# MILAB-IIT-CV/ATDN_vSLAM

Measured on AMD Instinct MI355X. Metric: frame-pairs/sec, KITTI 1241x376 odometry inference at 1/2/4/8 MI355X, higher is better.
Workload: dtype f32 via 3xf16 split MFMA (fp32 accumulate); 1 GPU; KITTI seq-03-shaped 376x1241 uint8 frames (resident in HBM) resized to 376x1232, GMA flow 12 GRU iters + CLVO head -> 6-DoF trajectory (BASELINE configs[1]); streams_per_gpu=2, gru_iters=12, parallelism=pairs sharded x1, one all-gather of 512-d features, replicated LSTM scan

## Files before the change

atdn_vslam_amd/_lib.py:

```python
import ctypes as C
import os

_HERE = os.path.dirname(os.path.abspath(__file__))
LIB_PATH = os.environ.get("ATDN_LIB_PATH") or os.path.join(_HERE, "libatdn_hip.so")

_f32p = C.POINTER(C.c_float)
_i64p = C.POINTER(C.c_int64)
_vp = C.c_void_p

SIGNATURES = {
    "atdn_version": (C.c_int, []),
    "atdn_last_error": (C.c_char_p, []),
    "atdn_gma_create": (C.c_int, [C.POINTER(_vp), C.c_int, C.c_int, C.c_int, C.c_int]),
    "atdn_gma_set_low_latency": (C.c_int, [_vp, C.c_int]),
    "atdn_gma_load": (C.c_int, [_vp, C.c_char_p, _vp, _i64p, C.c_int]),
    "atdn_gma_finalize": (C.c_int, [_vp]),
    "atdn_gma_forward": (C.c_int, [_vp, _vp, _vp, C.c_int, C.c_int, _vp, _vp, _vp, _vp]),
    "atdn_gma_forward_predictions": (C.c_int, [_vp, _vp, _vp, C.c_int, C.c_int, _vp, _vp, _vp]),
    "atdn_gma_forward_sequence": (C.c_int, [_vp, _vp, C.c_int, C.c_int, _vp, _vp, _vp, _vp]),
    "atdn_gma_forward_sequence_continued": (C.c_int, [_vp, _vp, C.c_int, C.c_int, _vp, _vp, _vp, _vp]),
    "atdn_gma_debug_read": (C.c_long, [_vp, C.c_char_p, _vp, C.c_long, _vp]),
    "atdn_gma_profile": (C.c_int, [_vp, C.c_int, C.c_int, C.c_int, _f32p, _vp]),
    "atdn_gma_profile_mode": (C.c_int, [_vp, C.c_int, C.c_int, C.c_int, C.c_int, _f32p, _vp]),
    "atdn_gma_set_range_probe": (C.c_int, [_vp, C.c_int]),
# ... 35 lines not shown
    "atdn_ingest_destroy": (None, [_vp]),
    "atdn_flow_pack_f16": (C.c_int, [_vp, C.c_int, C.c_int, C.c_int, C.c_int, C.c_int, _vp, _vp]),
    "atdn_flow_gather_clips": (C.c_int, [_vp, C.c_int, C.c_int, C.c_int, _vp, _vp, C.c_int, C.c_int, _vp, _vp]),
    "atdn_map_search": (C.c_int, [_vp, C.c_int, C.c_int, _vp, C.c_int, C.c_int, _vp, _vp, _vp]),
    "atdn_map_gather_images_u8": (C.c_int, [_vp, C.c_int, C.c_long, _vp, C.c_int, _vp, _vp]),
    "atdn_corr_lookup": (C.c_int, [_vp, _vp, _vp, _vp, C.c_int, C.c_int, C.c_int, _vp, _vp, C.c_int, _vp]),
    "atdn_corr_pyramid": (C.c_int, [_vp, _vp, C.c_int, C.c_int, C.c_int, C.c_int, _vp, _vp, _vp, _vp, _vp]),
    "atdn_corr_lookup_bricks": (C.c_int, [_vp, _vp, C.c_int, C.c_int, C.c_int, C.c_int, _vp, _vp, _vp, _vp, _vp, _vp, _vp, _vp,
                                          _vp, _vp]),
    "atdn_conv2d_nhwc": (C.c_int, [_vp, C.c_int, C.c_int, C.c_int, C.c_int, _vp, _vp, C.c_int, C.c_int, C.c_int,
                                   C.c_int, C.c_int, C.c_int, C.c_int, _vp, _vp]),
    "atdn_conv2d_nhwc_sf": (C.c_int, [_vp, C.c_int, C.c_int, C.c_int, C.c_int, _vp, _vp, C.c_int, C.c_int, C.c_int,
                                      C.c_int, C.c_int, C.c_int, _vp, _vp]),
    "atdn_conv2d_nhwc_sf_epi": (C.c_int, [_vp, C.c_int, C.c_int, C.c_int, C.c_int, _vp, _vp, C.c_int, C.c_int, C.c_int,
                                      C.c_int, C.c_int, C.c_int, C.c_int, _vp, _vp]),
}

GMA_STAGES = ("fnet", "corr", "pool", "cnet", "attention", "lookup", "motion_encoder", "aggregate", "gru_zr", "gru_q",
              "flow_head", "mask", "gru_ctx", "attn_logits", "agg_vt", "convc1", "gru_zr_v", "gru_q_v")

_lib = None


def lib():
    global _lib
    if _lib is None:
        if not os.path.exists(LIB_PATH):
            raise RuntimeError(
                "%s is missing: the HIP extension has not been built (python -m atdn_vslam_amd.build). "
                "There is no CPU fallback for the product path." % LIB_PATH)
# ... 31 lines not shown
```

atdn_vslam_amd/csrc/capi.hip:

```cpp
#include "../../include/atdn_hip.h"

#include <cmath>
#include <cstring>

#include "clvo.h"
#include "gma.h"
#include "vae.h"
#include "clvo_train.h"
#include "frontend.h"
#include "conv_sf.h"
#include "epilogues_sf.h"

namespace atdn {
extern template TileChoice conv_dispatch<MODE_TAP, EpiBias<ACT_NONE>>(const ConvShape&, EpiBias<ACT_NONE>, hipStream_t);
extern template TileChoice conv_dispatch<MODE_TAP, EpiBias<ACT_RELU>>(const ConvShape&, EpiBias<ACT_RELU>, hipStream_t);
extern template TileChoice conv_dispatch<MODE_ROW, EpiBias<ACT_NONE>>(const ConvShape&, EpiBias<ACT_NONE>, hipStream_t);
extern template TileChoice conv_dispatch<MODE_ROW, EpiBias<ACT_RELU>>(const ConvShape&, EpiBias<ACT_RELU>, hipStream_t);
extern template TileChoice conv_dispatch<MODE_TAP, EpiScale>(const ConvShape&, EpiScale, hipStream_t);

extern template TileChoice conv_sf_dispatch<EpiBias<ACT_NONE>>(const ConvShape&, float, EpiBias<ACT_NONE>, hipStream_t);
extern template TileChoice conv_sf_dispatch<SfBias<ACT_NONE>>(const ConvShape&, float, SfBias<ACT_NONE>, hipStream_t);

static thread_local std::string g_last_error;
void set_last_error(const std::string& msg) { g_last_error = msg; }
}
// ... 560 lines not shown
    (void)hipFree(tmp);
    A.release();
    throw;
  }
  (void)hipFree(tmp);
  A.release();
  ATDN_API_END
}

int atdn_conv2d_nhwc_sf(const float* src, int nimg, int H, int W, int Cin, const float* weight_host,
                        const float* bias_host, int Cout, int KH, int KW, int stride, int padH, int padW, float* dst,
                        void* stream) {
  return atdn_conv2d_nhwc_sf_epi(src, nimg, H, W, Cin, weight_host, bias_host, Cout, KH, KW, stride, padH, padW, 0, dst, stream);
}

}
```

atdn_vslam_amd/csrc/conv_sf6.h:

```cpp
#pragma once
#include <cstdlib>
#include <type_traits>
#include "conv_sf.h"

namespace atdn {

struct Conv2Geom {
  const float* src0; const float* src1;
  long sb0, sb1;
  int ld0, ld1, C0, C1;
  int H, W, Ho, Wo;
  int KH, KW, padH, padW;
  int PH, PW;
  int tiles_x, tiles_y;
  int nimg, ntile_n;
  const float* w; int ldw; int N;
  float wscale;
  const float* in_mean; const float* in_rstd;
};

inline bool conv_halo_eligible(const ConvShape& s) {
  if (s.stride != 1 || s.wb != 0) return false;
  return (s.KH == 3 && s.KW == 3) || (s.KH == 1 && s.KW == 5) || (s.KH == 5 && s.KW == 1);
}

template <class E, class = void> struct epi_gen6 : std::integral_constant<int, 0> {};
template <class E> struct epi_gen6<E, std::void_t<decltype(E::kGen6)>> : std::integral_constant<int, E::kGen6> {};
template <class E, class = void> struct EpiAux4 { struct type {}; };
template <class E> struct EpiAux4<E, std::void_t<typename E::Aux4>> { using type = typename E::Aux4; };
template <class E, class = void> struct epi_flowhead : std::false_type {};
template <class E> struct epi_flowhead<E, std::void_t<decltype(E::kFlowHead)>> : std::bool_constant<E::kFlowHead> {};
template <class E, class = void> struct epi_ring3 : std::false_type {};
template <class E> struct epi_ring3<E, std::void_t<decltype(E::kRing3)>> : std::bool_constant<E::kRing3> {};
template <class E, class = void> struct epi_rawacc : std::false_type {};
// ... 19 lines not shown
  constexpr int TM = TH * TW / 32 / WM, TN = BN / 32 / WN;
  static_assert(TM * WM * 32 == TH * TW && TN * WN * 32 == BN, "wave grid must tile the block");
  static_assert(32 % TW == 0 || TW % 32 == 0, "a 32-pixel MFMA row tile must cover whole tile rows");
  constexpr int NTAP = KH * KW;
  constexpr int RSTEP = NT / 8;
  constexpr int PROWS = (TH + KH - 1) * (TW + KW - 1);
  constexpr int PW = TW + KW - 1;
  constexpr int NP = (PROWS + RSTEP - 1) / RSTEP;
  constexpr int ROWB = 160;
  constexpr int RS = PW * ROWB;
  constexpr bool SWAP = epi_vec4<Epi>::value;
  constexpr int PSZ = (TH + KH - 1) * RS;
  __shared__ __attribute__((aligned(256))) char Pbytes[NIMG * PSZ];

  const int tid = threadIdx.x;
  const int tiles_img = g.tiles_x * g.tiles_y;
  const int nblk = g.nimg * tiles_img * g.ntile_n;
  const int id = xcd_remap(bidx, nblk);
  const int tile_n = id % g.ntile_n;
  const int tmg = id / g.ntile_n;
  const int img = tmg / tiles_img;
  const int tloc = tmg - img * tiles_img;
  const int ty0 = (tloc / g.tiles_x) * TH, tx0 = (tloc % g.tiles_x) * TW;
  const int n0 = tile_n * BN;
  const int lane = tid & 63, wave = tid >> 6;
#ifdef ATDN_CONV_STAMP
  constexpr int kStamp = conv_stamp_kind<Epi>::value;
  unsigned long long st_r0 = 0, st_t0 = 0, st_t1 = 0, st_t2 = 0, st_bar = 0;
  unsigned long long st_e_slab = 0, st_e_wait = 0, st_e_apply = 0;
  if constexpr (kStamp >= 0) { st_r0 = __builtin_amdgcn_s_memrealtime(); st_t0 = __builtin_amdgcn_s_memtime(); }
#endif

  const int jrow = (tid >> 3) & 7;
  const int s = tid & 7, r0 = !NORM ? tid >> 3 : ((tid >> 6) << 3) + 2 * (jrow & 1) + ((jrow >> 1) & 1) + 4 * (jrow >> 2);
  static_assert((TH + KH - 1) * RS / 16 <= 4096, "LDS offset field");
  unsigned pmeta[NP];
#pragma unroll
  for (int k = 0; k < NP; ++k) {
    const int prow = r0 + RSTEP * k;
    unsigned off = 0;
    const int py = prow / PW, px = prow - py * PW;
    if (prow < PROWS) {
      const int iy = ty0 - g.padH + py, ix = tx0 - g.padW + px;
      if ((unsigned)iy < (unsigned)g.H && (unsigned)ix < (unsigned)g.W) off = (unsigned)(iy * g.W + ix) + 1u;
    }
    pmeta[k] = (off << 12) | (unsigned)((py * RS + px * ROWB + 16 * s) >> 4);
    if (prow >= PROWS) pmeta[k] = pmeta[0];
  }
  const float* s0 = g.src0 + (long)img * g.sb0;
  const float* s1 = g.src1 ? g.src1 + (long)img * g.sb1 : nullptr;
  const int nck = (g.C0 + g.C1) >> 5;

  float4 pr[NP];
  auto fetch_patch = [&](int c) {
    const int cc = c << 5;
    const float* sp; int ld, co;
    if (cc < g.C0) { sp = s0; ld = g.ld0; co = cc; } else { sp = s1; ld = g.ld1; co = cc - g.C0; }
#pragma unroll
    for (int k = 0; k < NP; ++k)
      pr[k] = *reinterpret_cast<const float4*>(sp + (long)((pmeta[k] >> 12) ? (pmeta[k] >> 12) - 1 : 0) * ld + co + 4 * s);
  };
  auto store_patch = [&](int buf) {
// ... 22 lines not shown
    *reinterpret_cast<uint2*>(px + 64 + 8 * s) = make_uint2(l0, l1);
  };

  const int wm = wave / WN, wn = wave % WN;
  SfAcc acc[TM][TN];
#pragma unroll
  for (int i = 0; i < TM; ++i)
#pragma unroll
    for (int j = 0; j < TN; ++j) {
#pragma unroll
      for (int e = 0; e < 16; ++e) acc[i][j].b[e >> 3][(e >> 2) & 1][e & 3] = 0.f;
    }
  {
    const int n16 = lane & 15, g16 = lane >> 4;
    int a_off[TM];
#pragma unroll
    for (int i = 0; i < TM; ++i) a_off[i] = ((wm * TM + i) * 2) * RS + n16 * ROWB + 16 * g16;
    const char* Pb = Pbytes;
    const int nblk16 = (g.N + 15) >> 4;
    const float* wrow[TN][2];
#pragma unroll
    for (int j = 0; j < TN; ++j)
#pragma unroll
      for (int cb = 0; cb < 2; ++cb)
        wrow[j][cb] = g.w + (long)min(((n0 >> 4) + (wn * TN + j) * 2 + cb), nblk16 - 1) * (NTAP * nck) * 512 + lane * 4;
    constexpr int RT = (NTAP % 3 == 0 || epi_ring3<Epi>::value) ? 3 : 2;
    constexpr int CU = (NTAP % RT == 0) ? 1 : RT;
    constexpr int NS = CU * NTAP;
    static_assert(NS % RT == 0, "ring size must divide the K steps of an unrolled iteration");
    struct WFrag { f16x8 hi[TN][2], lo[TN][2]; };
    WFrag wr[RT];
    auto load_w = [&](WFrag& f, int c0, int st, int cb) __attribute__((always_inline)) {
// ... 10 lines not shown
#pragma unroll
    for (int st = 0; st < RT - 1; ++st) { load_w(wr[st], 0, st, 0); load_w(wr[st], 0, st, 1); }
    if constexpr ((ABL & 1) != 0) { load_w(wr[RT - 1], 0, RT - 1, 0); load_w(wr[RT - 1], 0, RT - 1, 1); }
    if constexpr (NORM) {
#pragma unroll
      for (int k = 0; k < NP; ++k) store_row_norm(0, k, nmu, nrs);
    } else {
      store_patch(0);
    }
    __syncthreads();
#ifdef ATDN_CONV_STAMP
    if constexpr (kStamp >= 0) st_t1 = __builtin_amdgcn_s_memtime();
#endif
    f16x8 ah[2][TM], al[2][TM];
    auto read_a = [&](int half, int tap) __attribute__((always_inline)) {
      const char* arow = Pb + (tap / KW + half) * RS + (tap % KW) * ROWB;
#pragma unroll
      for (int i = 0; i < TM; ++i) {
        ah[half][i] = *reinterpret_cast<const f16x8*>(arow + a_off[i]);
        if constexpr (!FAST) al[half][i] = *reinterpret_cast<const f16x8*>(arow + a_off[i] + 64);
      }
    };
    auto mfma_half = [&](int half, const WFrag& w) __attribute__((always_inline)) {
#pragma unroll
      for (int i = 0; i < TM; ++i)
#pragma unroll
        for (int j = 0; j < TN; ++j)
#pragma unroll
          for (int cb = 0; cb < 2; ++cb) {
            f32x4v c = acc[i][j].b[half][cb];
// ... 52 lines not shown
              else if (k - ((hs + 1 < NH) ? nds : 0) < nvm) __builtin_amdgcn_sched_group_barrier(0x020, 1, 0);
              else if (k - ((hs + 1 < NH) ? nds : 0) - nvm < ndw) __builtin_amdgcn_sched_group_barrier(0x200, 1, 0);
            }
          }
        }
        if (!(ABL & 2)) {
#ifdef ATDN_CONV_STAMP
          unsigned long long st_b0 = 0;
          if constexpr (kStamp >= 0) { asm volatile("s_waitcnt lgkmcnt(0)" ::: "memory"); st_b0 = __builtin_amdgcn_s_memtime(); }
#endif
          asm volatile("s_waitcnt lgkmcnt(0)\n\ts_barrier" ::: "memory");
#ifdef ATDN_CONV_STAMP
          if constexpr (kStamp >= 0) st_bar += __builtin_amdgcn_s_memtime() - st_b0;
#endif
          Pb = Pbytes + ((c + 1) & 1) * PSZ;
        }
        if (!(ABL & 4)) read_a(0, 0);
      }
    }
  }

#ifdef ATDN_CONV_STAMP
  if constexpr (kStamp >= 0) st_t2 = __builtin_amdgcn_s_memtime();
  auto stamp_out = [&]() __attribute__((always_inline)) {
    if constexpr (kStamp >= 0) {
      asm volatile("s_waitcnt vmcnt(0) lgkmcnt(0)" ::: "memory");
      const unsigned long long t3 = __builtin_amdgcn_s_memtime(), r1 = __builtin_amdgcn_s_memrealtime();
      const unsigned hw = __builtin_amdgcn_s_getreg((31 << 11) | 4), xcc = __builtin_amdgcn_s_getreg((31 << 11) | 20);
      if (wave == 0 && lane == 0 && bidx < ATDN_CONV_STAMP_SLOTS) {
        unsigned long long* o = atdn_conv_stamps_dev[kStamp * 2 + (KH == 5 ? 1 : 0)][bidx];
        o[0] = st_r0; o[1] = r1; o[2] = st_t1 - st_t0; o[3] = st_t2 - st_t1; o[4] = st_bar; o[5] = t3 - st_t2;
        o[6] = ((unsigned long long)xcc << 32) | hw; o[7] = t3 - st_t0;
        o[8] = st_e_slab; o[9] = st_e_wait; o[10] = st_e_apply; o[11] = 0;
      }
    }
  };
#endif
  if constexpr (KH != 3 || !Epi::kStats) __builtin_amdgcn_s_setprio(0);
  if constexpr (NORM) sf_report(norm_sat);
  if constexpr ((ABL & 8) != 0) {
    float tot = 0.f;
#pragma unroll
    for (int i = 0; i < TM; ++i)
#pragma unroll
      for (int j = 0; j < TN; ++j)
#pragma unroll
        for (int e = 0; e < 16; ++e) tot += acc[i][j].b[e >> 3][(e >> 2) & 1][e & 3];
    if (tot == 1.2345e-30f) ep(img, 0, 0, tot);
    return;
  }
  if constexpr (SWAP) {
    static_assert(NW * 32 * LDS_LD * 4 <= NIMG * PSZ, "transpose slabs must fit in the patch images");
    __syncthreads();
    float* tb = reinterpret_cast<float*>(Pbytes) + wave * (32 * LDS_LD);
    const int trow = lane >> 3, tcol = (lane & 7) * 4;
    auto tile_pixel = [&](int i, int q) {
      const int p = (wm * TM + i) * 32 + 8 * q + trow;
      const int oy = ty0 + p / TW, ox = tx0 + p % TW;
      if constexpr ((ABL & 16) != 0) return p;
      return (oy < g.Ho && ox < g.Wo) ? oy * g.Wo + ox : -1;
    };
    constexpr bool RAW = epi_rawacc<Epi>::value && !epi_flowhead<Epi>::value;
    auto slab_write = [&](const SfAcc& a) __attribute__((always_inline)) {
      const float sc = RAW ? 1.0f : g.wscale;
#pragma unroll
      for (int hh = 0; hh < 2; ++hh)
#pragma unroll
        for (int cb = 0; cb < 2; ++cb)
          *reinterpret_cast<float4*>(tb + (16 * hh + (lane & 15)) * LDS_LD + 16 * cb + 4 * (lane >> 4)) =
              RAW ? make_float4(a.b[hh][cb][0], a.b[hh][cb][1], a.b[hh][cb][2], a.b[hh][cb][3])
                  : make_float4(a.b[hh][cb][0] * sc, a.b[hh][cb][1] * sc, a.b[hh][cb][2] * sc, a.b[hh][cb][3] * sc);
    };
    if constexpr (epi_flowhead<Epi>::value) {
      static_assert(!epi_flowhead<Epi>::value || (WM == 1 && TN == 1 && TW == 16), "one block holds all output channels of its pixels");
      constexpr int RP = 20;
// ... 47 lines not shown
              d1 = __builtin_amdgcn_mfma_f32_16x16x32_f16(w2l[1], xh[pb], d1, 0, 0, 0);
            }
            d0 = __builtin_amdgcn_mfma_f32_16x16x32_f16(w2h[0], xh[pb], d0, 0, 0, 0);
            d1 = __builtin_amdgcn_mfma_f32_16x16x32_f16(w2h[1], xh[pb], d1, 0, 0, 0);
            float* rp = tb + (16 * pb + n16) * RP;
            *reinterpret_cast<float4*>(rp + 4 * g16) = make_float4(d0[0] * ep.w2inv, d0[1] * ep.w2inv, d0[2] * ep.w2inv, d0[3] * ep.w2inv);
            if (g16 == 0) *reinterpret_cast<float2*>(rp + 16) = make_float2(d1[0] * ep.w2inv, d1[1] * ep.w2inv);
          }
          __syncthreads();
          for (int idx = tid; idx < 32 * 18; idx += NT) {
            const int px = idx / 18, u = idx - px * 18;
            const float* rq = reinterpret_cast<const float*>(Pbytes) + px * RP + u;
            float sum = 0.f;
#pragma unroll
            for (int w = 0; w < NW; ++w) sum += rq[w * (32 * LDS_LD)];
            const int p = i * 32 + px;
            const int oy = ty0 + p / TW, ox = tx0 + p % TW;
            if (oy < g.Ho && ox < g.Wo)
              ep.G[(long)(n0 / (NW * 32)) * ep.gstride + ((long)img * ep.npix + (long)oy * g.Wo + ox) * 18 + u] = sum;
          }
          __syncthreads();
        }
        sf_report(sat);
        return;
      }
    }
    struct NoAux {};
    using AuxT = typename std::conditional<Epi::kPrefetch, typename EpiAux4<Epi>::type, NoAux>::type;
    constexpr bool PIPE = Epi::kPrefetch && sizeof(AuxT) <= 2 * sizeof(float4);
    AuxT aux_next[PIPE ? 4 : 1];
    bool clamped = false;
    if constexpr (PIPE) {
      const int nb0 = n0 + (wn * TN) * 32 + tcol;
#pragma unroll
// ... 93 lines not shown
#pragma unroll
  for (int j = 0; j < TN; ++j)
#pragma unroll
    for (int cs = 0; cs < NSET; ++cs) {
      const int n = min(n0 + (wn * TN + j) * 32 + col_of(cs), g.N - 1);
      biasj[j][cs] = 0.f;
      if constexpr (Epi::kStats) biasj[j][cs] = ep.bias[n];
      if constexpr (epi_bias_arg<Epi>::value) colj[j][cs] = ep.col(n);
    }
#pragma unroll
  for (int i = 0; i < TM; ++i) {
    const int pbase = (wm * TM + i) * 32;
    int mm[NPX];
#pragma unroll
    for (int e = 0; e < NPX; ++e) {
      const int p = pbase + pix_of(e);
      const int oy = ty0 + p / TW, ox = tx0 + p % TW;
      mm[e] = (oy < g.Ho && ox < g.Wo) ? oy * g.Wo + ox : -1;
    }
    int cnt = 0;
    unsigned mo[NPX];
    if constexpr (Epi::kStats) {
#pragma unroll
      for (int e = 0; e < NPX; ++e) {
        cnt += mm[e] >= 0 ? 1 : 0;
        mo[e] = (unsigned)max(mm[e], 0) * (unsigned)ep.ld;
      }
      cnt += __shfl_xor(cnt, 16);
      cnt += __shfl_xor(cnt, 32);
      cnt = __builtin_amdgcn_readfirstlane(cnt);
    }
    const bool full = cnt == 32;
    const float inv_cnt = 1.0f / (float)(cnt > 0 ? cnt : 1);
// ... 71 lines not shown
}

template <int TH, int TW, int BN, int WM, int WN, int KH, int KW, class Epi, bool FAST = false, bool NORM = false, int ABL = 0>
__global__ __launch_bounds__(WM * WN * 64, 1) void conv_sf6_kernel(const Conv2Geom g, const Epi ep) {
  conv_sf6_body<TH, TW, BN, WM, WN, KH, KW, Epi, FAST, NORM, ABL>(g, ep, (int)blockIdx.x);
}

__device__ __forceinline__ Conv2Geom conv2_geom_pick(const Conv2Geom& a, const Conv2Geom& b, bool s) {
  Conv2Geom g;
  g.src0 = s ? b.src0 : a.src0; g.src1 = s ? b.src1 : a.src1; g.sb0 = s ? b.sb0 : a.sb0; g.sb1 = s ? b.sb1 : a.sb1;
  g.ld0 = s ? b.ld0 : a.ld0; g.ld1 = s ? b.ld1 : a.ld1; g.C0 = s ? b.C0 : a.C0; g.C1 = s ? b.C1 : a.C1;
  g.H = s ? b.H : a.H; g.W = s ? b.W : a.W; g.Ho = s ? b.Ho : a.Ho; g.Wo = s ? b.Wo : a.Wo;
  g.KH = s ? b.KH : a.KH; g.KW = s ? b.KW : a.KW; g.padH = s ? b.padH : a.padH; g.padW = s ? b.padW : a.padW;
  g.PH = s ? b.PH : a.PH; g.PW = s ? b.PW : a.PW; g.tiles_x = s ? b.tiles_x : a.tiles_x; g.tiles_y = s ? b.tiles_y : a.tiles_y;
  g.nimg = s ? b.nimg : a.nimg; g.ntile_n = s ? b.ntile_n : a.ntile_n;
  g.w = s ? b.w : a.w; g.ldw = s ? b.ldw : a.ldw; g.N = s ? b.N : a.N; g.wscale = s ? b.wscale : a.wscale;
  g.in_mean = nullptr; g.in_rstd = nullptr;
  return g;
}
template <int TH, int TW, int BN, int WM, int WN, int KH, int KW, class Epi, bool FAST = false>
__global__ __launch_bounds__(WM * WN * 64, 1) void conv_sf6_pair_kernel(const Conv2Geom g0, const Conv2Geom g1, const Epi ep0,
                                                                        const Epi ep1, const int nblk0, const int start1) {
  const int b = (int)blockIdx.x;
  if (b >= nblk0 && b < start1) return;
  const bool second = b >= start1;
  const Conv2Geom g = conv2_geom_pick(g0, g1, second);
  const Epi ep = Epi::pick(ep0, ep1, second);
  conv_sf6_body<TH, TW, BN, WM, WN, KH, KW, Epi, FAST, false, 0>(g, ep, second ? b - start1 : b);
}

// ... 3 lines not shown
  ATDN_CHECK(s.KH == KH && s.KW == KW && s.stride == 1, "kernel shape does not match the instantiation");
  Conv2Geom g{};
  g.src0 = s.src0; g.src1 = s.src1; g.sb0 = s.sb0; g.sb1 = s.sb1; g.ld0 = s.ld0; g.ld1 = s.ld1;
  g.C0 = s.C0; g.C1 = s.C1; g.H = s.H; g.W = s.W;
  g.KH = s.KH; g.KW = s.KW; g.padH = s.padH; g.padW = s.padW;
  g.Ho = conv_out(s.H, s.KH, 1, s.padH); g.Wo = conv_out(s.W, s.KW, 1, s.padW);
  g.PH = TH + s.KH - 1; g.PW = TW + s.KW - 1;
  ATDN_CHECK(s.C0 % 32 == 0 && s.C1 % 32 == 0 && s.C0 > 0 && s.ld0 % 4 == 0, "TAP-mode channel constraints");
  ATDN_CHECK(s.ldw % 4 == 0 && s.ldw >= s.KH * s.KW * (s.C0 + s.C1), "weight rows too short");
  ATDN_CHECK(!epi_vec4<Epi>::value || !Epi::kPrefetch || s.N % 4 == 0, "channel-vector epilogue with operand loads needs N % 4 == 0");
  ATDN_CHECK((long)s.H * s.W < (1L << 20) - 1, "image too large for the packed patch descriptor");
  ATDN_CHECK((long)g.Ho * g.Wo * 1024L * 4L <= (1L << 32) && s.ld0 <= 1024 && s.ld1 <= 1024 && s.N <= 1024,
             "per-image slice of 4 GB or more: the 32-bit epilogue offsets would wrap");
  g.tiles_x = cdiv(g.Wo, TW); g.tiles_y = cdiv(g.Ho, TH);
  g.nimg = s.nimg; g.ntile_n = cdiv(s.N, BN);
  g.w = s.wfrag16; g.ldw = s.ldw; g.N = s.N; g.wscale = wscale;
  g.in_mean = s.in_mean; g.in_rstd = s.in_rstd;
  ATDN_CHECK(NORM == (s.in_mean != nullptr) && (!NORM || (s.in_rstd && s.C1 == 0 && s.ld0 == s.C0)),
             "normalise-on-load: one dense fp32 source with its mean / rstd");
  ATDN_CHECK(g.w != nullptr, "missing weight copy for this kernel");
  return g;
}

template <int TH, int BN, int WM, int WN, int KH, int KW, class Epi, bool FAST = false, bool NORM = false, int ABL = 0>
inline void launch_conv_sf6(const ConvShape& s, float wscale, Epi ep, hipStream_t st) {
  constexpr int TW = 16;
  const Conv2Geom g = conv_sf6_geom<TH, BN, WM, WN, KH, KW, Epi, FAST, NORM, ABL>(s, wscale);
  set_groups(ep, g.tiles_x * g.tiles_y * (TH * TW / 32));
  const int nblk = g.nimg * g.tiles_x * g.tiles_y * g.ntile_n;
  hipLaunchKernelGGL((conv_sf6_kernel<TH, TW, BN, WM, WN, KH, KW, Epi, FAST, NORM, ABL>), dim3(nblk), dim3(WM * WN * 64), 0, st, g, ep);
  ATDN_HIP(hipGetLastError());
}

template <int TH, int BN, int WM, int WN, int KH, int KW, class Epi, bool FAST>
inline void launch_conv_sf6_pair(const ConvShape& s0, float wscale0, Epi ep0, const ConvShape& s1, float wscale1, Epi ep1,
                                 hipStream_t st) {
  constexpr int TW = 16;
  static_assert(!Epi::kStats, "the pair launch serves plain-store epilogues");
  const Conv2Geom g0 = conv_sf6_geom<TH, BN, WM, WN, KH, KW, Epi, FAST, false, 0>(s0, wscale0);
  const Conv2Geom g1 = conv_sf6_geom<TH, BN, WM, WN, KH, KW, Epi, FAST, false, 0>(s1, wscale1);
  const int nblk0 = g0.nimg * g0.tiles_x * g0.tiles_y * g0.ntile_n;
  const int start1 = (nblk0 + 7) / 8 * 8;
  const int nblk1 = g1.nimg * g1.tiles_x * g1.tiles_y * g1.ntile_n;
  hipLaunchKernelGGL((conv_sf6_pair_kernel<TH, TW, BN, WM, WN, KH, KW, Epi, FAST>), dim3(start1 + nblk1), dim3(WM * WN * 64), 0, st,
                     g0, g1, ep0, ep1, nblk0, start1);
  ATDN_HIP(hipGetLastError());
}


inline int conv_sf6_block_width_3x3(const ConvShape& s) {
  const int Ho = conv_out(s.H, s.KH, 1, s.padH), Wo = conv_out(s.W, s.KW, 1, s.padW);
  const long tiles = (long)s.nimg * cdiv(Wo, 16) * cdiv(Ho, 8);
  int bn = 64;
  if (s.N <= 32) bn = 32;
  else if (s.N == 96) bn = 96;
  else {
    int best = cdiv(s.N, 64) * 64;
    for (int c : {128, 256})
// ... 129 lines not shown
```

atdn_vslam_amd/csrc/gma.hip:

```cpp
#include "gma.h"
#include "small_convs.h"
#include "conv_sf.h"
#include "epilogues_sf.h"

namespace atdn { const float* zero_line(); }

namespace atdn {

extern template TileChoice conv_dispatch<MODE_TAP, EpiBias<ACT_NONE>>(const ConvShape&, EpiBias<ACT_NONE>, hipStream_t);
extern template TileChoice conv_dispatch<MODE_TAP, EpiBias<ACT_RELU>>(const ConvShape&, EpiBias<ACT_RELU>, hipStream_t);
extern template TileChoice conv_dispatch<MODE_ROW, EpiBias<ACT_RELU>>(const ConvShape&, EpiBias<ACT_RELU>, hipStream_t);
extern template TileChoice conv_dispatch<MODE_TAP, EpiBiasStats>(const ConvShape&, EpiBiasStats, hipStream_t);
extern template TileChoice conv_dispatch<MODE_ROW, EpiBiasStats>(const ConvShape&, EpiBiasStats, hipStream_t);
extern template TileChoice conv_dispatch<MODE_TAP, EpiBiasReluAddRelu>(const ConvShape&, EpiBiasReluAddRelu, hipStream_t);
extern template TileChoice conv_dispatch<MODE_TAP, EpiContextSplit>(const ConvShape&, EpiContextSplit, hipStream_t);
extern template TileChoice conv_dispatch<MODE_TAP, EpiScale>(const ConvShape&, EpiScale, hipStream_t);
extern template TileChoice conv_dispatch<MODE_TAP, EpiQK>(const ConvShape&, EpiQK, hipStream_t);
extern template TileChoice conv_dispatch<MODE_TAP, EpiStoreT>(const ConvShape&, EpiStoreT, hipStream_t);
extern template TileChoice conv_dispatch<MODE_TAP, EpiAggregate>(const ConvShape&, EpiAggregate, hipStream_t);
extern template TileChoice conv_dispatch<MODE_TAP, EpiGruZR>(const ConvShape&, EpiGruZR, hipStream_t);
extern template TileChoice conv_dispatch<MODE_TAP, EpiGruQ>(const ConvShape&, EpiGruQ, hipStream_t);
extern template TileChoice conv_dispatch<MODE_TAP, EpiFlowDelta>(const ConvShape&, EpiFlowDelta, hipStream_t);

extern template TileChoice conv_dispatch<MODE_ROW, SfBias<ACT_RELU>>(const ConvShape&, SfBias<ACT_RELU>, hipStream_t);
// ... 301 lines not shown
  z_.alloc(n8 * 128); rh_.alloc(n8 * 128); fh_.alloc(n8 * 256); mask_.alloc(n8 * 576);
  if (sf) fhG_.alloc(2 * n8 * 18);
  coords1_.alloc(n8 * 2); flow4_.alloc(n8 * 4);
  if (sf) for (int p = 0; p < 2; ++p) { pre_zr_[p].alloc(n8 * 256); pre_q_[p].alloc(n8 * 128); }
  ATDN_HIP(hipMemset(corrfeat_.p, 0, corrfeat_.n * sizeof(float)));
  ATDN_HIP(hipMemset(vT_.p, 0, vT_.n * sizeof(float)));
  ATDN_HIP(hipMemset(attn_.p, 0, attn_.n * sizeof(float)));
  ATDN_HIP(hipMemset(flow4_.p, 0, flow4_.n * sizeof(float)));
  ATDN_HIP(hipDeviceSynchronize());
  ws_bytes_ = 0;
  DeviceBuf* all[] = {&img4_, &enc_[0], &enc_[1], &enc_[2], &enc_[3], &fmap_, &psum_, &pm2_, &pyr_[0], &pyr_[1], &pyr_[2],
                      &pyr_[3], &h_[0], &h_[1], &x_, &qk_, &attn_, &vT_, &corrfeat_, &cor1_, &corflo_, &flo1_, &z_,
                      &rh_, &fh_, &mask_, &coords1_, &flow4_};
  for (auto* b : all) ws_bytes_ += (size_t)b->n * sizeof(float);
  (void)zero_line();
  sf_counter_attach();
  ATDN_HIP(hipStreamCreateWithFlags(&cap_stream_, hipStreamNonBlocking));
  ready_ = true;
}

void GmaNet::run_encoder(const EncoderWeights& E, bool instance, int nimg, hipStream_t st, float** out_buf, int* outH,
                         int* outW) {
  int h = conv_out(H, 7, 2, 3), w = conv_out(W, 7, 2, 3);
  float* P = enc_[0].p; float* Q = enc_[1].p; float* R = enc_[2].p;
  auto stats_conv = [&](auto mode_tag, const PackedConv& L, const float* src, int ld, int ih, int iw, int stride,
                        int pad, float* dst, int slot) {
    constexpr int MODE = decltype(mode_tag)::value;
    ConvShape s = conv_shape(L, src, ld, (long)ih * iw * ld, nimg, ih, iw, stride, pad, pad);
    const int oh = conv_out(ih, L.KH, stride, pad), ow = conv_out(iw, L.KW, stride, pad);
    EpiBiasStats ep{L.b, dst, (long)oh * ow * L.N, L.N, psum_.p, pm2_.p, 0};
// ... 604 lines not shown
```

include/atdn_hip.h:

```cpp
#ifndef ATDN_HIP_H
#define ATDN_HIP_H

#include <stddef.h>
#include <stdint.h>

#ifdef __cplusplus
extern "C" {
#endif

typedef struct atdn_gma atdn_gma;
typedef struct atdn_clvo atdn_clvo;
typedef struct atdn_vae atdn_vae;
typedef struct atdn_clvo_trainer atdn_clvo_trainer;

int atdn_version(void);
const char* atdn_last_error(void);


#define ATDN_PRECISION_F32 0
#define ATDN_PRECISION_SPLIT_F16 1
#define ATDN_PRECISION_F16 2
int atdn_gma_create(atdn_gma** out, int H, int W, int max_batch, int precision);

int atdn_gma_set_low_latency(atdn_gma* h, int on);
// ... 101 lines not shown
int atdn_corr_lookup_bricks(const float* fmap1, const float* fmap2, int B, int H8, int W8, int C, const float* coords,
                            float* pyr0, float* pyr1, float* pyr2, float* pyr3, float* samples,
                            const float* convc1_weight_host, const float* convc1_bias_host, float* cor1, void* stream);

int atdn_conv2d_nhwc(const float* src, int nimg, int H, int W, int Cin, const float* weight_host,
                     const float* bias_host, int Cout, int KH, int KW, int stride, int padH, int padW, int relu,
                     float* dst, void* stream);

int atdn_conv2d_nhwc_sf(const float* src, int nimg, int H, int W, int Cin, const float* weight_host,
                        const float* bias_host, int Cout, int KH, int KW, int stride, int padH, int padW, float* dst,
                        void* stream);
int atdn_conv2d_nhwc_sf_epi(const float* src, int nimg, int H, int W, int Cin, const float* weight_host,
                            const float* bias_host, int Cout, int KH, int KW, int stride, int padH, int padW, int sf_store,
                            float* dst, void* stream);

#ifdef __cplusplus
}
#endif
#endif
```

Baseline: 418.1 frame-pairs/s.

## Use precomputed fitted tile plans for ragged edges in halo-patch convs

Adds a host-built tile plan that covers the output image with full 16xTH tiles plus reshaped edge tiles sized to the remainder strips, cached on device per shape. For plain-store epilogues without stats or normalisation, the halo-patch conv kernel reads its tile geometry from the plan and uses variable patch strides and pixel-slot mappings. The aim is to cut the wasted MFMA work and patch loads that partially empty edge tiles spend on out-of-range pixels. In exchange each block does a plan load, float-reciprocal index math and more address arithmetic, and the A-fragment addressing becomes more complex.

```diff
diff --git a/atdn_vslam_amd/_lib.py b/atdn_vslam_amd/_lib.py
--- a/atdn_vslam_amd/_lib.py
+++ b/atdn_vslam_amd/_lib.py
@@ -73,6 +73,7 @@
                                       C.c_int, C.c_int, C.c_int, _vp, _vp]),
     "atdn_conv2d_nhwc_sf_epi": (C.c_int, [_vp, C.c_int, C.c_int, C.c_int, C.c_int, _vp, _vp, C.c_int, C.c_int, C.c_int,
                                       C.c_int, C.c_int, C.c_int, C.c_int, _vp, _vp]),
+    "atdn_conv_tile_plan": (C.c_int, [C.c_int, C.c_int, C.c_int, C.c_int, C.c_int, C.POINTER(C.c_int), C.c_int, C.POINTER(C.c_int)]),
 }
 
 GMA_STAGES = ("fnet", "corr", "pool", "cnet", "attention", "lookup", "motion_encoder", "aggregate", "gru_zr", "gru_q",
diff --git a/atdn_vslam_amd/csrc/capi.hip b/atdn_vslam_amd/csrc/capi.hip
--- a/atdn_vslam_amd/csrc/capi.hip
+++ b/atdn_vslam_amd/csrc/capi.hip
@@ -9,6 +9,7 @@
 #include "clvo_train.h"
 #include "frontend.h"
 #include "conv_sf.h"
+#include "conv_tile_plan.h"
 #include "epilogues_sf.h"
 
 namespace atdn {
@@ -599,4 +600,17 @@
   return atdn_conv2d_nhwc_sf_epi(src, nimg, H, W, Cin, weight_host, bias_host, Cout, KH, KW, stride, padH, padW, 0, dst, stream);
 }
 
-}
+int atdn_conv_tile_plan(int Ho, int Wo, int TH, int KH, int KW, int* tiles, int capacity, int* count) {
+  ATDN_API_BEGIN
+  ATDN_CHECK(Ho >= 1 && Wo >= 1 && count && capacity >= 0 && (tiles || capacity == 0), "bad argument");
+  ATDN_CHECK(TH == 4 || TH == 8 || TH == 12, "tile heights of the halo-patch kernels: 4, 8, 12");
+  ATDN_CHECK((KH == 3 && KW == 3) || (KH == 1 && KW == 5) || (KH == 5 && KW == 1), "kernel shapes of the halo-patch kernels: 3x3, 1x5, 5x1");
+  const std::vector<ConvTile> plan = conv_tile_plan(Ho, Wo, TH, KH, KW);
+  *count = (int)plan.size();
+  for (int i = 0; i < (int)plan.size() && i < capacity; ++i) {
+    tiles[4 * i + 0] = plan[i].y0; tiles[4 * i + 1] = plan[i].x0; tiles[4 * i + 2] = plan[i].h; tiles[4 * i + 3] = plan[i].w;
+  }
+  ATDN_API_END
+}
+
+}
diff --git a/atdn_vslam_amd/csrc/conv_sf6.h b/atdn_vslam_amd/csrc/conv_sf6.h
--- a/atdn_vslam_amd/csrc/conv_sf6.h
+++ b/atdn_vslam_amd/csrc/conv_sf6.h
@@ -2,6 +2,7 @@
 #include <cstdlib>
 #include <type_traits>
 #include "conv_sf.h"
+#include "conv_tile_plan.h"
 
 namespace atdn {
 
@@ -17,7 +18,10 @@
   const float* w; int ldw; int N;
   float wscale;
   const float* in_mean; const float* in_rstd;
+  const ConvTile* plan; int ntiles;
 };
+
+template <class Epi, bool NORM, int ABL> struct conv_sf6_fit : std::bool_constant<!Epi::kStats && !NORM && ABL == 0> {};
 
 inline bool conv_halo_eligible(const ConvShape& s) {
   if (s.stride != 1 || s.wb != 0) return false;
@@ -67,14 +71,43 @@
   __shared__ __attribute__((aligned(256))) char Pbytes[NIMG * PSZ];
 
   const int tid = threadIdx.x;
-  const int tiles_img = g.tiles_x * g.tiles_y;
+  constexpr bool FIT = conv_sf6_fit<Epi, NORM, ABL>::value;
+  const int tiles_img = FIT ? g.ntiles : g.tiles_x * g.tiles_y;
   const int nblk = g.nimg * tiles_img * g.ntile_n;
   const int id = xcd_remap(bidx, nblk);
   const int tile_n = id % g.ntile_n;
   const int tmg = id / g.ntile_n;
   const int img = tmg / tiles_img;
   const int tloc = tmg - img * tiles_img;
-  const int ty0 = (tloc / g.tiles_x) * TH, tx0 = (tloc % g.tiles_x) * TW;
+  int ty0, tx0, t_h = TH, t_w = TW, t_wh = TW, t_hh = TH / 2, t_ry = 2, t_dy = 1, t_dx = 0, pwf = PW;
+  float inv_wh = 1.0f / TW;
+  auto load_tile = [&]() __attribute__((always_inline)) {
+    const int4 ta = reinterpret_cast<const int4*>(g.plan)[2 * tloc], tb4 = reinterpret_cast<const int4*>(g.plan)[2 * tloc + 1];
+    ty0 = ta.x; tx0 = ta.y; t_h = ta.z; t_w = ta.w; t_wh = tb4.x; t_hh = tb4.y;
+    t_ry = tb4.z & 255; t_dy = (tb4.z >> 8) & 255; t_dx = (tb4.z >> 16) & 255;
+    inv_wh = __int_as_float(__builtin_amdgcn_readfirstlane(__float_as_int(__builtin_amdgcn_rcpf((float)t_wh))));
+  };
+  if constexpr (FIT) {
+    load_tile();
+    pwf = (t_dx ? 2 * t_wh : t_w) + KW - 1;
+  } else {
+    ty0 = (tloc / g.tiles_x) * TH; tx0 = (tloc % g.tiles_x) * TW;
+  }
+  const int rs = FIT ? pwf * ROWB : RS;
+  const int hoff = FIT ? t_dy * rs + t_dx * ROWB : RS;
+  const int nprow = FIT ? ((t_ry == 2 ? (t_h + 1) & ~1 : t_h) + KH - 1) * pwf : PROWS;
+  const float inv_pw = __builtin_amdgcn_rcpf((float)pwf);
+  auto slot_pixel = [&](int I, int half, int n) __attribute__((always_inline)) {
+    if constexpr (FIT) {
+      const int u = I * 16 + n;
+      const int q = (int)(((float)u + 0.5f) * inv_wh), r = u - q * t_wh;
+      const int y = q * t_ry + half * t_dy, x = r + half * t_dx;
+      return (q < t_hh && y < t_h && x < t_w) ? (ty0 + y) * g.Wo + tx0 + x : -1;
+    } else {
+      const int oy = ty0 + I * (32 / TW) + half, ox = tx0 + n;
+      return (oy < g.Ho && ox < g.Wo) ? oy * g.Wo + ox : -1;
+    }
+  };
   const int n0 = tile_n * BN;
   const int lane = tid & 63, wave = tid >> 6;
 #ifdef ATDN_CONV_STAMP
@@ -92,13 +125,13 @@
   for (int k = 0; k < NP; ++k) {
     const int prow = r0 + RSTEP * k;
     unsigned off = 0;
-    const int py = prow / PW, px = prow - py * PW;
-    if (prow < PROWS) {
+    const int py = FIT ? (int)(((float)prow + 0.5f) * inv_pw) : prow / PW, px = prow - py * pwf;
+    if (prow < nprow) {
       const int iy = ty0 - g.padH + py, ix = tx0 - g.padW + px;
       if ((unsigned)iy < (unsigned)g.H && (unsigned)ix < (unsigned)g.W) off = (unsigned)(iy * g.W + ix) + 1u;
     }
-    pmeta[k] = (off << 12) | (unsigned)((py * RS + px * ROWB + 16 * s) >> 4);
-    if (prow >= PROWS) pmeta[k] = pmeta[0];
+    pmeta[k] = (off << 12) | (unsigned)((py * rs + px * ROWB + 16 * s) >> 4);
+    if (prow >= nprow) pmeta[k] = pmeta[0];
   }
   const float* s0 = g.src0 + (long)img * g.sb0;
   const float* s1 = g.src1 ? g.src1 + (long)img * g.sb1 : nullptr;
@@ -151,8 +184,26 @@
   {
     const int n16 = lane & 15, g16 = lane >> 4;
     int a_off[TM];
-#pragma unroll
-    for (int i = 0; i < TM; ++i) a_off[i] = ((wm * TM + i) * 2) * RS + n16 * ROWB + 16 * g16;
+    int a_cur[TM];
+#pragma unroll
+    for (int i = 0; i < TM; ++i) {
+      if constexpr (FIT) {
+        const int u = (wm * TM + i) * 16 + n16;
+        const int q = (int)(((float)u + 0.5f) * inv_wh), r = u - q * t_wh;
+        a_cur[i] = min(q, t_hh - 1) * t_ry * rs + r * ROWB + 16 * g16;
+        a_off[i] = 0;
+      } else {
+        a_off[i] = ((wm * TM + i) * 2) * RS + n16 * ROWB + 16 * g16;
+        a_cur[i] = 0;
+      }
+    }
+    auto a_step = [&](int d) __attribute__((always_inline)) {
+#pragma unroll
+      for (int i = 0; i < TM; ++i) {
+        if constexpr (Epi::kPrefetch) { a_cur[i] += d; asm("" : "+v"(a_cur[i])); }
+        else asm("v_add_u32 %0, %1, %0" : "+v"(a_cur[i]) : "s"(d));
+      }
+    };
     const char* Pb = Pbytes;
     const int nblk16 = (g.N + 15) >> 4;
     const float* wrow[TN][2];
@@ -193,6 +244,17 @@
 #endif
     f16x8 ah[2][TM], al[2][TM];
     auto read_a = [&](int half, int tap) __attribute__((always_inline)) {
+      if constexpr (FIT) {
+        if (half == 1) a_step(hoff);
+        else if (tap > 0) a_step(tap % KW == 0 ? rs - hoff : -hoff);
+#pragma unroll
+        for (int i = 0; i < TM; ++i) {
+          const char* ap = Pbytes + a_cur[i] + (tap % KW) * ROWB;
+          ah[half][i] = *reinterpret_cast<const f16x8*>(ap);
+          if constexpr (!FAST) al[half][i] = *reinterpret_cast<const f16x8*>(ap + 64);
+        }
+        return;
+      }
       const char* arow = Pb + (tap / KW + half) * RS + (tap % KW) * ROWB;
 #pragma unroll
       for (int i = 0; i < TM; ++i) {
@@ -275,6 +337,7 @@
           if constexpr (kStamp >= 0) st_bar += __builtin_amdgcn_s_memtime() - st_b0;
 #endif
           Pb = Pbytes + ((c + 1) & 1) * PSZ;
+          if constexpr (FIT) a_step((((c + 1) & 1) ? PSZ : -PSZ) - (KH - 1) * rs - hoff);
         }
         if (!(ABL & 4)) read_a(0, 0);
       }
@@ -298,6 +361,7 @@
   };
 #endif
   if constexpr (KH != 3 || !Epi::kStats) __builtin_amdgcn_s_setprio(0);
+  if constexpr (FIT) load_tile();
   if constexpr (NORM) sf_report(norm_sat);
   if constexpr ((ABL & 8) != 0) {
     float tot = 0.f;
@@ -316,10 +380,8 @@
     float* tb = reinterpret_cast<float*>(Pbytes) + wave * (32 * LDS_LD);
     const int trow = lane >> 3, tcol = (lane & 7) * 4;
     auto tile_pixel = [&](int i, int q) {
-      const int p = (wm * TM + i) * 32 + 8 * q + trow;
-      const int oy = ty0 + p / TW, ox = tx0 + p % TW;
-      if constexpr ((ABL & 16) != 0) return p;
-      return (oy < g.Ho && ox < g.Wo) ? oy * g.Wo + ox : -1;
+      if constexpr ((ABL & 16) != 0) return (wm * TM + i) * 32 + 8 * q + trow;
+      return slot_pixel(wm * TM + i, q >> 1, 8 * (q & 1) + trow);
     };
     constexpr bool RAW = epi_rawacc<Epi>::value && !epi_flowhead<Epi>::value;
     auto slab_write = [&](const SfAcc& a) __attribute__((always_inline)) {
@@ -397,10 +459,8 @@
             float sum = 0.f;
 #pragma unroll
             for (int w = 0; w < NW; ++w) sum += rq[w * (32 * LDS_LD)];
-            const int p = i * 32 + px;
-            const int oy = ty0 + p / TW, ox = tx0 + p % TW;
-            if (oy < g.Ho && ox < g.Wo)
-              ep.G[(long)(n0 / (NW * 32)) * ep.gstride + ((long)img * ep.npix + (long)oy * g.Wo + ox) * 18 + u] = sum;
+            const int m = slot_pixel(i, px >> 4, px & 15);
+            if (m >= 0) ep.G[(long)(n0 / (NW * 32)) * ep.gstride + ((long)img * ep.npix + m) * 18 + u] = sum;
           }
           __syncthreads();
         }
@@ -524,9 +584,7 @@
     int mm[NPX];
 #pragma unroll
     for (int e = 0; e < NPX; ++e) {
-      const int p = pbase + pix_of(e);
-      const int oy = ty0 + p / TW, ox = tx0 + p % TW;
-      mm[e] = (oy < g.Ho && ox < g.Wo) ? oy * g.Wo + ox : -1;
+      mm[e] = slot_pixel(pbase >> 5, pix_of(e) >> 4, pix_of(e) & 15);
     }
     int cnt = 0;
     unsigned mo[NPX];
@@ -628,6 +686,7 @@
   g.KH = s ? b.KH : a.KH; g.KW = s ? b.KW : a.KW; g.padH = s ? b.padH : a.padH; g.padW = s ? b.padW : a.padW;
   g.PH = s ? b.PH : a.PH; g.PW = s ? b.PW : a.PW; g.tiles_x = s ? b.tiles_x : a.tiles_x; g.tiles_y = s ? b.tiles_y : a.tiles_y;
   g.nimg = s ? b.nimg : a.nimg; g.ntile_n = s ? b.ntile_n : a.ntile_n;
+  g.plan = s ? b.plan : a.plan; g.ntiles = s ? b.ntiles : a.ntiles;
   g.w = s ? b.w : a.w; g.ldw = s ? b.ldw : a.ldw; g.N = s ? b.N : a.N; g.wscale = s ? b.wscale : a.wscale;
   g.in_mean = nullptr; g.in_rstd = nullptr;
   return g;
@@ -661,6 +720,8 @@
              "per-image slice of 4 GB or more: the 32-bit epilogue offsets would wrap");
   g.tiles_x = cdiv(g.Wo, TW); g.tiles_y = cdiv(g.Ho, TH);
   g.nimg = s.nimg; g.ntile_n = cdiv(s.N, BN);
+  g.plan = nullptr; g.ntiles = g.tiles_x * g.tiles_y;
+  if constexpr (conv_sf6_fit<Epi, NORM, ABL>::value) g.plan = conv_tile_plan_device(g.Ho, g.Wo, TH, KH, KW, &g.ntiles);
   g.w = s.wfrag16; g.ldw = s.ldw; g.N = s.N; g.wscale = wscale;
   g.in_mean = s.in_mean; g.in_rstd = s.in_rstd;
   ATDN_CHECK(NORM == (s.in_mean != nullptr) && (!NORM || (s.in_rstd && s.C1 == 0 && s.ld0 == s.C0)),
@@ -674,7 +735,7 @@
   constexpr int TW = 16;
   const Conv2Geom g = conv_sf6_geom<TH, BN, WM, WN, KH, KW, Epi, FAST, NORM, ABL>(s, wscale);
   set_groups(ep, g.tiles_x * g.tiles_y * (TH * TW / 32));
-  const int nblk = g.nimg * g.tiles_x * g.tiles_y * g.ntile_n;
+  const int nblk = g.nimg * g.ntiles * g.ntile_n;
   hipLaunchKernelGGL((conv_sf6_kernel<TH, TW, BN, WM, WN, KH, KW, Epi, FAST, NORM, ABL>), dim3(nblk), dim3(WM * WN * 64), 0, st, g, ep);
   ATDN_HIP(hipGetLastError());
 }
@@ -686,9 +747,9 @@
   static_assert(!Epi::kStats, "the pair launch serves plain-store epilogues");
   const Conv2Geom g0 = conv_sf6_geom<TH, BN, WM, WN, KH, KW, Epi, FAST, false, 0>(s0, wscale0);
   const Conv2Geom g1 = conv_sf6_geom<TH, BN, WM, WN, KH, KW, Epi, FAST, false, 0>(s1, wscale1);
-  const int nblk0 = g0.nimg * g0.tiles_x * g0.tiles_y * g0.ntile_n;
+  const int nblk0 = g0.nimg * g0.ntiles * g0.ntile_n;
   const int start1 = (nblk0 + 7) / 8 * 8;
-  const int nblk1 = g1.nimg * g1.tiles_x * g1.tiles_y * g1.ntile_n;
+  const int nblk1 = g1.nimg * g1.ntiles * g1.ntile_n;
   hipLaunchKernelGGL((conv_sf6_pair_kernel<TH, TW, BN, WM, WN, KH, KW, Epi, FAST>), dim3(start1 + nblk1), dim3(WM * WN * 64), 0, st,
                      g0, g1, ep0, ep1, nblk0, start1);
   ATDN_HIP(hipGetLastError());
diff --git a/atdn_vslam_amd/csrc/conv_tile_plan.h b/atdn_vslam_amd/csrc/conv_tile_plan.h
--- /dev/null
+++ b/atdn_vslam_amd/csrc/conv_tile_plan.h
@@ -0,0 +1,80 @@
+#pragma once
+#include <vector>
+
+namespace atdn {
+
+struct ConvTile {
+  int y0, x0, h, w;
+  int wh, hh;
+  int pk;
+  int pad;
+};
+
+inline int conv_tile_patch_rows(int TH, int KH, int KW) { return (TH + KH - 1) * (16 + KW - 1); }
+
+inline bool conv_tile_shape(int h, int w, int TH, int KH, int KW, ConvTile* t) {
+  if (h < 1 || w < 1 || h * w > TH * 16) return false;
+  int wh, hh, ry, dy, dx, he = h, we = w;
+  if (w == 16 && h <= TH) { wh = 16; he = (h + 1) & ~1; hh = he / 2; ry = 2; dy = 1; dx = 0; }
+  else if (h % 2 == 0) { wh = w; hh = h / 2; ry = 1; dy = h / 2; dx = 0; }
+  else { wh = (w + 1) / 2; hh = h; ry = 1; dy = 0; dx = wh; we = 2 * wh; }
+  if (ry == 1 && hh * wh > TH * 8) return false;
+  if ((he + KH - 1) * (we + KW - 1) > conv_tile_patch_rows(TH, KH, KW)) return false;
+  if (dy > 255 || dx > 255) return false;
+  t->h = h; t->w = w; t->wh = wh; t->hh = hh; t->pk = ry | (dy << 8) | (dx << 16); t->pad = 0;
+  return true;
+}
+
+inline void conv_tile_extent(const ConvTile& t, int* he, int* we) {
+  const int ry = t.pk & 255, dx = (t.pk >> 16) & 255;
+  *he = ry == 2 ? (t.h + 1) & ~1 : t.h;
+  *we = dx ? 2 * t.wh : t.w;
+}
+
+inline std::vector<ConvTile> conv_tile_plan(int Ho, int Wo, int TH, int KH, int KW) {
+  const int nx = Wo / 16, rw = Wo % 16, ny = Ho / TH, rh = Ho % TH;
+  auto put = [&](std::vector<ConvTile>& v, int y0, int x0, int h, int w) {
+    ConvTile t{};
+    if (!conv_tile_shape(h, w, TH, KH, KW, &t)) return false;
+    t.y0 = y0; t.x0 = x0;
+    v.push_back(t);
+    return true;
+  };
+  std::vector<ConvTile> grid;
+  for (int y = 0; y < Ho; y += TH)
+    for (int x = 0; x < Wo; x += 16) put(grid, y, x, Ho - y < TH ? Ho - y : TH, Wo - x < 16 ? Wo - x : 16);
+  if (rw == 0 && rh == 0) return grid;
+  auto cut_rows = [&](std::vector<ConvTile>& v, int y0, int x0, int H, int w) {
+    for (int y = 0; y < H;) {
+      int h = H - y < TH * 16 ? H - y : TH * 16;
+      while (h > 1 && !put(v, y0 + y, x0, h, w)) --h;
+      if (h == 1) put(v, y0 + y, x0, 1, w);
+      y += h;
+    }
+  };
+  auto cut_cols = [&](std::vector<ConvTile>& v, int y0, int x0, int h, int Wd) {
+    for (int x = 0; x < Wd;) {
+      int w = Wd - x < TH * 16 ? Wd - x : TH * 16;
+      while (w > 1 && !put(v, y0, x0 + x, h, w)) --w;
+      if (w == 1) put(v, y0, x0 + x, h, 1);
+      x += w;
+    }
+  };
+  std::vector<ConvTile> cand[2];
+  for (int c = 0; c < 2; ++c) {
+    std::vector<ConvTile>& v = cand[c];
+    for (int y = 0; y < ny; ++y)
+      for (int x = 0; x < nx; ++x) put(v, y * TH, x * 16, TH, 16);
+    const bool strip_owns_corner = c == 0;
+    if (rw) cut_rows(v, 0, nx * 16, strip_owns_corner ? Ho : ny * TH, rw);
+    if (rh) cut_cols(v, ny * TH, 0, rh, strip_owns_corner ? nx * 16 : Wo);
+  }
+  const std::vector<ConvTile>* best = &grid;
+  for (int c = 0; c < 2; ++c)
+    if (cand[c].size() < best->size()) best = &cand[c];
+  return *best;
+}
+
+const ConvTile* conv_tile_plan_device(int Ho, int Wo, int TH, int KH, int KW, int* count);
+
+}
diff --git a/atdn_vslam_amd/csrc/conv_tile_plan.hip b/atdn_vslam_amd/csrc/conv_tile_plan.hip
--- /dev/null
+++ b/atdn_vslam_amd/csrc/conv_tile_plan.hip
@@ -0,0 +1,35 @@
+#include "conv_tile_plan.h"
+
+#include <array>
+#include <map>
+#include <mutex>
+
+#include "common.h"
+
+namespace atdn {
+
+const ConvTile* conv_tile_plan_device(int Ho, int Wo, int TH, int KH, int KW, int* count) {
+  static std::mutex mu;
+  static std::map<std::array<int, 6>, std::pair<ConvTile*, int>> plans;
+  int dev = 0;
+  ATDN_HIP(hipGetDevice(&dev));
+  const std::array<int, 6> key = {dev, Ho, Wo, TH, KH, KW};
+  std::lock_guard<std::mutex> lock(mu);
+  auto it = plans.find(key);
+  if (it == plans.end()) {
+    const std::vector<ConvTile> plan = conv_tile_plan(Ho, Wo, TH, KH, KW);
+    ATDN_CHECK(!plan.empty(), "empty tile plan");
+    ConvTile* d = nullptr;
+    ATDN_HIP(hipMalloc(&d, plan.size() * sizeof(ConvTile)));
+    hipError_t e = hipMemcpy(d, plan.data(), plan.size() * sizeof(ConvTile), hipMemcpyHostToDevice);
+    if (e != hipSuccess) {
+      (void)hipFree(d);
+      ATDN_HIP(e);
+    }
+    it = plans.emplace(key, std::make_pair(d, (int)plan.size())).first;
+  }
+  *count = it->second.second;
+  return it->second.first;
+}
+
+}
diff --git a/atdn_vslam_amd/csrc/gma.hip b/atdn_vslam_amd/csrc/gma.hip
--- a/atdn_vslam_amd/csrc/gma.hip
+++ b/atdn_vslam_amd/csrc/gma.hip
@@ -1,6 +1,7 @@
 #include "gma.h"
 #include "small_convs.h"
 #include "conv_sf.h"
+#include "conv_tile_plan.h"
 #include "epilogues_sf.h"
 
 namespace atdn { const float* zero_line(); }
@@ -339,6 +340,14 @@
                       &rh_, &fh_, &mask_, &coords1_, &flow4_};
   for (auto* b : all) ws_bytes_ += (size_t)b->n * sizeof(float);
   (void)zero_line();
+  if (sf) {
+    for (int d : {2, 4, 8})
+      for (int th : {4, 8, 12})
+        for (int k = 0; k < 3; ++k) {
+          int cnt = 0;
+          (void)conv_tile_plan_device(H / d, W / d, th, k == 0 ? 3 : (k == 1 ? 1 : 5), k == 0 ? 3 : (k == 1 ? 5 : 1), &cnt);
+        }
+  }
   sf_counter_attach();
   ATDN_HIP(hipStreamCreateWithFlags(&cap_stream_, hipStreamNonBlocking));
   ready_ = true;
diff --git a/include/atdn_hip.h b/include/atdn_hip.h
--- a/include/atdn_hip.h
+++ b/include/atdn_hip.h
@@ -139,6 +139,8 @@
                             const float* bias_host, int Cout, int KH, int KW, int stride, int padH, int padW, int sf_store,
                             float* dst, void* stream);
 
+int atdn_conv_tile_plan(int Ho, int Wo, int TH, int KH, int KW, int* tiles, int capacity, int* count);
+
 #ifdef __cplusplus
 }
 #endif
```

New measurement: 419.3 frame-pairs/s, median of 6. No clear change (+0.3%).
